# SamsungLabs/cloud_transformers

Hardware: AMD Instinct MI355X
Metric: points/sec fwd+bwd MHCT, 4096-pt batch, 1/2/4/8 MI355X; % HBM roofline (higher is better)
Workload: dtype f32; 1 GPU; north-star op-level: B=8 clouds x N=4096 pts, H=64 heads, C=16 feat/head, 2D grid W=32, reduce=max, keys=tanh(randn), seed 1234+rank; step = Splat fwd, Slice fwd, Slice bwd, Splat bwd (key cotangents summed); per_gpu_batch=8, parallelism=replica-sharded clouds x1 (no collective), world_size_seen=1, hip_graph=True, steps_per_graph=10

## Files before the change

### cloud_transformers_amd/csrc/ct_raster_bwd_fused.h

```cpp
#pragma once

typedef unsigned ct_u4 __attribute__((ext_vector_type(4)));
struct StreamBuf {
  __amdgpu_buffer_rsrc_t r;
};
constexpr int kBufNt = 2;
__device__ __forceinline__ StreamBuf stream_buf(const float* base, unsigned bytes) {
  StreamBuf b;
  b.r = __builtin_amdgcn_make_buffer_rsrc((void*)base, 0, (int)bytes, 0x00020000);
  return b;
}
__device__ __forceinline__ float4 buf_ld_stream4(const StreamBuf& b, unsigned voff, unsigned soff) {
  const ct_u4 v = __builtin_amdgcn_raw_buffer_load_b128(b.r, (int)voff, (int)soff, kBufNt);
  return make_float4(__uint_as_float(v.x), __uint_as_float(v.y), __uint_as_float(v.z), __uint_as_float(v.w));
}
__device__ __forceinline__ float buf_ld_stream(const StreamBuf& b, unsigned voff, unsigned soff) {
  return __uint_as_float(__builtin_amdgcn_raw_buffer_load_b32(b.r, (int)voff, (int)soff, kBufNt));
}
__device__ __forceinline__ void buf_st_stream4(const StreamBuf& b, unsigned voff, unsigned soff, float4 v) {
  const ct_u4 t = {__float_as_uint(v.x), __float_as_uint(v.y), __float_as_uint(v.z), __float_as_uint(v.w)};
  __builtin_amdgcn_raw_buffer_store_b128(t, b.r, (int)voff, (int)soff, kBufNt);
}
__device__ __forceinline__ void buf_st_stream(const StreamBuf& b, unsigned voff, unsigned soff, float v) {
  __builtin_amdgcn_raw_buffer_store_b32(__float_as_uint(v), b.r, (int)voff, (int)soff, kBufNt);
}

template <bool HAS_PAD, int WT, int NT = 0, int CT = 0>
__global__ void __launch_bounds__(kSortThreads) slice_splat_bwd_kernel(RasterArgs a_arg, GridW<2> g_arg) {
  const GridW<2> g = grid2_of<WT>(g_arg);
  RasterArgs a = a_arg;
  if constexpr (NT > 0) a.N = NT;
  if constexpr (CT > 0) a.C = CT;
  extern __shared__ __align__(16) unsigned char lds_raw[];
  const int G = WT ? WT * WT : g.G, W1 = WT ? WT : g.W[1], N = a.N, C = a.C;
  const SortLds L = sort_lds(G, N, C);
  float4* T4 = (float4*)(lds_raw + L.tile);
  int* acc = (int*)(lds_raw + L.acc);
  float4* ZG = (float4*)(lds_raw + L.tile);
  float4* Sg = (float4*)(lds_raw + L.stage);
  const float2* AB = (const float2*)(lds_raw + L.ab);
  unsigned* s_max = (unsigned*)(lds_raw + L.misc);
  unsigned* s_k = s_max + C;
  int* s_tie = (int*)(s_k + 1);
  const int b = blockIdx.z;
  const size_t bh = (size_t)b * a.H + blockIdx.y;
  const int tid = threadIdx.x;
  const int off[4] = {0, W1, 1, W1 + 1};
  const bool has = (tid << 2) < N;
  const int n0 = has ? (tid << 2) : 0;
  const int ngroups = C >> 2;
  const float* const feat = a.tile_in2;

  float gq[4][4];
  float fq[4][4];
  float cvq[4];
  const unsigned ln0 = (unsigned)n0;
  const unsigned pt_row = (unsigned)N * 4u, cell_row = (unsigned)G * 4u;
  const StreamBuf b_src = stream_buf(a.src + bh * C * (size_t)N, (unsigned)C * pt_row);
  const StreamBuf b_fea = stream_buf(feat + bh * C * (size_t)N, (unsigned)C * pt_row);
  const StreamBuf b_dst = stream_buf(a.dst + bh * C * (size_t)N, (unsigned)C * pt_row);
  const StreamBuf b_cnv = stream_buf(a.tile_in + bh * C * (size_t)G, (unsigned)C * cell_row);
  const StreamBuf b_gz = stream_buf(a.tile_out + bh * C * (size_t)G, (unsigned)C * cell_row);
  const unsigned vo_pt = ln0 * 4u, vo_cell = tid < G ? (unsigned)tid * 4u : 0u;
  auto request1 = [&](int grp, int cj) {
    const float4 t = buf_ld_stream4(b_src, vo_pt, (unsigned)(grp * 4 + cj) * pt_row);
    gq[cj][0] = t.x; gq[cj][1] = t.y; gq[cj][2] = t.z; gq[cj][3] = t.w;
    cvq[cj] = buf_ld_stream(b_cnv, vo_cell, (unsigned)(grp * 4 + cj) * cell_row);
  };
  auto request_feat1 = [&](int grp, int cj) {
    const float4 t = buf_ld_stream4(b_fea, vo_pt, (unsigned)(grp * 4 + cj) * pt_row);
    fq[cj][0] = t.x; fq[cj][1] = t.y; fq[cj][2] = t.z; fq[cj][3] = t.w;
  };
  PlaneKeys PK;
  load_plane_keys(a, g, W1, bh, PK);
  SortedPlane S;
  float pv[4];
#pragma unroll
  for (int i = 0; i < 4; ++i) pv[i] = (HAS_PAD && has) ? ct_load_pad(a.pad, a.pad_dtype, (size_t)b * N + n0 + i) : 1.0f;

  sort_plane(a, PK, G, W1, sort_ptrs(lds_raw, L, C), C, S, nullptr, [&]() {
#pragma unroll
    for (int cj = 0; cj < 4; ++cj) request1(0, cj);
  });
  uint2* const s_cell = (uint2*)(lds_raw + L.mark);
  s_cell[tid] = make_uint2((unsigned)PK.base[0] | (unsigned)PK.base[1] << 16, (unsigned)PK.base[2] | (unsigned)PK.base[3] << 16);
  for (int i = tid; i < G; i += kSortThreads) ((int4*)acc)[i] = make_int4(0, 0, 0, 0);
  if (tid == 0) Sg[N] = make_float4(0.0f, 0.0f, 0.0f, 0.0f);
  if (tid < 4) s_tie[tid] = 0;
  const float Kf = (float)(*s_k);

  float gsx[2][kItemLen], gsy[2][kItemLen];
#pragma unroll
  for (int u = 0; u < 2; ++u)
#pragma unroll
    for (int j = 0; j < kItemLen; ++j) gsx[u][j] = gsy[u][j] = 0.0f;
  float gs[4][2];
#pragma unroll
  for (int i = 0; i < 4; ++i) gs[i][0] = gs[i][1] = 0.0f;
  unsigned cell01 = ((unsigned)S.cell[0] & 0xffffu) | (unsigned)S.cell[1] << 16;
  unsigned long long tied = 0ull;

  auto group = [&](const int grp, auto more) {
    const int ch0 = grp * 4;
    asm volatile("" : "+v"(S.rk01), "+v"(S.rk23), "+v"(cell01));
    const int cell[2] = {(int)(short)(cell01 & 0xffffu), (int)cell01 >> 16};
#pragma unroll
    for (int cj = 0; cj < 4; ++cj) {
      float m = 0.0f;
#pragma unroll
      for (int i = 0; i < 4; ++i) {
        float x = HAS_PAD ? gq[cj][i] * pv[i] : gq[cj][i];
        x = has ? x : 0.0f;
        gq[cj][i] = x;
        x = fabsf(x);
        m = fmaxf(m, (x < __builtin_inff()) ? x : __builtin_inff());
      }
      const unsigned mb = wave_max_u32(__float_as_uint(m));
      if ((tid & 63) == 0) atomicMax(&s_max[ch0 + cj], mb);
    }
    if (has) {
      const unsigned rk[4] = {S.rk01 & kRankMask, (S.rk01 >> 16) & kRankMask, S.rk23 & kRankMask, (S.rk23 >> 16) & kRankMask};
#pragma unroll
      for (int i = 0; i < 4; ++i) Sg[rk[i]] = make_float4(gq[0][i], gq[1][i], gq[2][i], gq[3][i]);
    }
    if (tid < G) T4[tid] = make_float4(cvq[0], cvq[1], cvq[2], cvq[3]);
    __syncthreads();

    float iq[4];
    bool any_float = false;
#pragma unroll
    for (int cj = 0; cj < 4; ++cj) {
      float q;
      bool fixed;
      fx_quantum(__uint_as_float(s_max[ch0 + cj]) * Kf, q, iq[cj], fixed);
      if (!fixed) {
        iq[cj] = 0.0f;
        any_float = true;
      }
      iq[cj] = __uint_as_float(__builtin_amdgcn_readfirstlane(__float_as_uint(iq[cj])));
    }
    auto item = [&](auto U) {
      constexpr int u = decltype(U)::value;
      int Y = cell[u] < 0 ? 0 : cell[u];
      asm volatile("" : "+v"(S.ent8[u][0]), "+v"(S.ent8[u][1]), "+v"(Y));
      float4 cv[4];
#pragma unroll
      for (int v = 0; v < 4; ++v) cv[v] = T4[Y + off[v]];
      float4 xn = *(const float4*)((const unsigned char*)Sg + 2u * CT_E8(S, u, 0));
      float2 wn = *(const float2*)((const unsigned char*)AB + CT_E8(S, u, 0));
      ct_f2 s01[4], s23[4];
#pragma unroll
      for (int v = 0; v < 4; ++v) s01[v] = s23[v] = ct_f2{0.0f, 0.0f};
#pragma unroll
      for (int j = 0; j < kItemLen; ++j) {
        if constexpr (u == 0) request_feat1(grp, j);
        const float4 x = xn;
        const float2 wf = wn;
        if (j + 1 < kItemLen) {
          xn = *(const float4*)((const unsigned char*)Sg + 2u * CT_E8(S, u, j + 1));
          wn = *(const float2*)((const unsigned char*)AB + CT_E8(S, u, j + 1));
        }
        const ct_f2 x01 = {x.x, x.y}, x23 = {x.z, x.w};
        const float w1x = wf.x, w1y = wf.y, w0x = 1.0f - w1x, w0y = 1.0f - w1y;
        const float cw[4] = {w0x * w0y, w1x * w0y, w0x * w1y, w1x * w1y};
        float gw[4];
#pragma unroll
        for (int v = 0; v < 4; ++v) {
          const ct_f2 cwv = {cw[v], cw[v]};
          s01[v] = __builtin_elementwise_fma(x01, cwv, s01[v]);
          s23[v] = __builtin_elementwise_fma(x23, cwv, s23[v]);
          const ct_f2 c01 = {cv[v].x, cv[v].y}, c23 = {cv[v].z, cv[v].w};
          const ct_f2 pr = __builtin_elementwise_fma(c23, x23, c01 * x01);
          gw[v] = pr.x + pr.y;
        }
        gsx[u][j] = __builtin_fmaf(gw[3] - gw[2], w1y, __builtin_fmaf(gw[1] - gw[0], w0y, gsx[u][j]));
        gsy[u][j] = __builtin_fmaf(gw[3] - gw[1], w1x, __builtin_fmaf(gw[2] - gw[0], w0x, gsy[u][j]));
        asm volatile("" : "+v"(gsx[u][j]), "+v"(gsy[u][j]));
        CT_SB;
      }
      if (cell[u] >= 0) {
        const ct_f2 iq01 = {iq[0], iq[1]}, iq23 = {iq[2], iq[3]};
        int* Tc = acc + Y;
#pragma unroll
        for (int v = 0; v < 4; ++v) {
          const ct_f2 a01 = s01[v] * iq01, a23 = s23[v] * iq23;
          atomicAdd(Tc + off[v], cvt_rpi(a01.x));
          atomicAdd(Tc + G + off[v], cvt_rpi(a01.y));
          atomicAdd(Tc + 2 * G + off[v], cvt_rpi(a23.x));
          atomicAdd(Tc + 3 * G + off[v], cvt_rpi(a23.y));
        }
      }
      CT_SB;
    };
    item(std::integral_constant<int, 0>{});
    if (cell[1] >= 0) item(std::integral_constant<int, 1>{});
    if (any_float) {
#pragma unroll 1
      for (int cj = 0; cj < 4; ++cj)
        if (iq[cj] == 0.0f) scatter_float_channel<HAS_PAD>(a, g, bh, b, ch0 + cj, (float*)(acc + cj * G), 1, 0);
    }
    __syncthreads();

    float4 zc = make_float4(0.0f, 0.0f, 0.0f, 0.0f);
    float gv[4] = {0.0f, 0.0f, 0.0f, 0.0f};
    if (tid < G) {
      zc = T4[tid];
#pragma unroll
      for (int cj = 0; cj < 4; ++cj) {
        float q, iqd;
        bool fixed;
        fx_quantum(__uint_as_float(s_max[ch0 + cj]) * Kf, q, iqd, fixed);
        const int r = acc[cj * G + tid];
        gv[cj] = fixed ? (float)r * q : __int_as_float(r);
        buf_st_stream(b_gz, vo_cell, (unsigned)(ch0 + cj) * cell_row, gv[cj]);
      }
    }
    const unsigned zw[4] = {__float_as_uint(zc.x), __float_as_uint(zc.y), __float_as_uint(zc.z), __float_as_uint(zc.w)};
    {
      int nzt = 0;
#pragma unroll
      for (int k = 0; k < 4; ++k) nzt += (zw[k] != 0u);
      nzt = wave_sum_i32(nzt);
      if ((tid & 63) == 0 && nzt) atomicAdd(&s_tie[(grp & 1) * 2], nzt);
    }
    __syncthreads();
    if (tid < G) {
      ZG[tid] = make_float4(__uint_as_float(zw[0] ? zw[0] : kNoMatch), __uint_as_float(zw[1] ? zw[1] : kNoMatch), gv[0], gv[1]);
      ZG[G + tid] = make_float4(__uint_as_float(zw[2] ? zw[2] : kNoMatch), __uint_as_float(zw[3] ? zw[3] : kNoMatch), gv[2], gv[3]);
    }
    __syncthreads();

    int nm = 0;
    if (has) {
      const uint2 bc = s_cell[tid];
      const unsigned rk[4] = {S.rk01 & kRankMask, (S.rk01 >> 16) & kRankMask, S.rk23 & kRankMask, (S.rk23 >> 16) & kRankMask};
      const int pbase[4] = {(int)(bc.x & 0xffffu), (int)(bc.x >> 16), (int)(bc.y & 0xffffu), (int)(bc.y >> 16)};
#pragma unroll
      for (int i = 0; i < 4; ++i) {
        if constexpr (decltype(more)::value) request1(grp + 1, i);
        const float2 w1 = AB[rk[i]];
        Pt2 p;
        p.w1x = w1.x; p.w1y = w1.y; p.w0x = 1.0f - w1.x; p.w0y = 1.0f - w1.y;
        p.base = pbase[i];
        p.cw[0] = p.w0x * p.w0y; p.cw[1] = p.w1x * p.w0y; p.cw[2] = p.w0x * p.w1y; p.cw[3] = p.w1x * p.w1y;
        float gw[4] = {0.0f, 0.0f, 0.0f, 0.0f};
#pragma unroll
        for (int pr = 0; pr < 2; ++pr) {
          const float4* Zp = ZG + (size_t)pr * G + p.base;
          const float xa = HAS_PAD ? fq[2 * pr][i] * pv[i] : fq[2 * pr][i];
          const float xb = HAS_PAD ? fq[2 * pr + 1][i] * pv[i] : fq[2 * pr + 1][i];
          ct_f4 zg[4];
#pragma unroll
          for (int v = 0; v < 4; ++v) zg[v] = *(const ct_f4*)(Zp + off[v]);
#pragma unroll
          for (int v = 0; v < 4; ++v) asm volatile("" : "+v"(zg[v].x), "+v"(zg[v].y), "+v"(zg[v].z), "+v"(zg[v].w));
          float gfa = 0.0f, gfb = 0.0f;
#pragma unroll
          for (int v = 0; v < 4; ++v) {
            const unsigned ba = __float_as_uint(xa * p.cw[v]), bb = __float_as_uint(xb * p.cw[v]);
            const bool ma = ba == __float_as_uint(zg[v].x), mb = bb == __float_as_uint(zg[v].y);
            nm += (int)ma;
            nm += (int)mb;
            asm volatile("" : "+v"(nm));
            const float ga = ma ? zg[v].z : 0.0f, gb = mb ? zg[v].w : 0.0f;
            gfa = __builtin_fmaf(ga, p.cw[v], gfa);
            gfb = __builtin_fmaf(gb, p.cw[v], gfb);
            gw[v] = __builtin_fmaf(gb, xb, __builtin_fmaf(ga, xa, gw[v]));
          }
          fq[2 * pr][i] = HAS_PAD ? gfa * pv[i] : gfa;
          fq[2 * pr + 1][i] = HAS_PAD ? gfb * pv[i] : gfb;
        }
        gs[i][0] = __builtin_fmaf(gw[3] - gw[2], p.w1y, __builtin_fmaf(gw[1] - gw[0], p.w0y, gs[i][0]));
        gs[i][1] = __builtin_fmaf(gw[3] - gw[1], p.w1x, __builtin_fmaf(gw[2] - gw[0], p.w0x, gs[i][1]));
        asm volatile("" : "+v"(gs[i][0]), "+v"(gs[i][1]), "+v"(fq[0][i]), "+v"(fq[1][i]), "+v"(fq[2][i]), "+v"(fq[3][i]));
        __builtin_amdgcn_sched_barrier(0);
      }
#pragma unroll
      for (int cj = 0; cj < 4; ++cj)
        buf_st_stream4(b_dst, vo_pt, (unsigned)(ch0 + cj) * pt_row, make_float4(fq[cj][0], fq[cj][1], fq[cj][2], fq[cj][3]));
    } else if constexpr (decltype(more)::value) {
#pragma unroll
      for (int cj = 0; cj < 4; ++cj) request1(grp + 1, cj);
    }
    nm = wave_sum_i32(nm);
    if ((tid & 63) == 0 && nm) atomicAdd(&s_tie[(grp & 1) * 2 + 1], nm);
    __syncthreads();
    const int* tw = s_tie + (grp & 1) * 2;
    if (tw[0] != tw[1]) tied |= 1ull << grp;
    if (tid < 2) s_tie[((grp & 1) ^ 1) * 2 + tid] = 0;
    int zero;
    asm volatile("v_mov_b32 %0, 0" : "=v"(zero));
    if (tid < G) ((int4*)acc)[tid] = make_int4(zero, zero, zero, zero);
  };
  int grp = 0;
  for (; grp + 1 < ngroups; ++grp) group(grp, std::true_type{});
  group(grp, std::false_type{});

  if (tied != 0ull) {
    __builtin_amdgcn_fence(__ATOMIC_RELEASE, "workgroup");
    asm volatile("s_waitcnt vmcnt(0)" ::: "memory");
    __syncthreads();
    __builtin_amdgcn_fence(__ATOMIC_ACQUIRE, "workgroup");
    RasterArgs a2 = a;
    a2.src = feat;
    PtRows R;
    R.Nr = N; R.so = 0; R.wt = false;
    for (int gi = 0; gi < ngroups; ++gi) {
      if (!((tied >> gi) & 1ull)) continue;
      const int cabs = gi << 2;
      const float* zin = a.tile_in + (bh * C + cabs) * (size_t)G;
      const float* gin = a.tile_out + (bh * C + cabs) * (size_t)G;
      __syncthreads();
      {
        int nz_unused = 0;
        unsigned long long nzp_unused = 0ull;
        unsigned xzp_unused = 0u;
        stage_tile_pairs<false>(ZG, zin, gin, 2, G, nz_unused, nzp_unused, xzp_unused);
      }
      __syncthreads();
      if (has) {
        const float* const key0 = a.pos.keys + bh * 2 * (size_t)N;
        const float4 tx = *(const float4*)(key0 + ln0), ty = *(const float4*)(key0 + N + ln0);
        const float kx[4] = {tx.x, tx.y, tx.z, tx.w}, ky[4] = {ty.x, ty.y, ty.z, ty.w};
        int nm_unused = 0;
        unsigned u0 = 0u, u1 = 0u;
        splat_bwd_quad<HAS_PAD, true, WT, true>(a2, g, ZG, bh, b, cabs, 4, n0, R, kx, ky, gs, nm_unused, u0, u1, false);
      }
    }
    __syncthreads();
  }

  float2* Gs = (float2*)Sg;
#pragma unroll
  for (int u = 0; u < 2; ++u)
#pragma unroll
    for (int j = 0; j < kItemLen; ++j)
      *(float2*)((unsigned char*)Gs + CT_E8(S, u, j)) = make_float2(gsx[u][j], gsy[u][j]);
  __syncthreads();
  if (has) {
    const unsigned rw[4] = {S.rk01 & 0xffffu, S.rk01 >> 16, S.rk23 & 0xffffu, S.rk23 >> 16};
    float2 gk[4];
#pragma unroll
    for (int i = 0; i < 4; ++i) {
      gk[i] = Gs[rw[i] & kRankMask];
      gk[i].x *= (rw[i] & kInsideX) ? 1.0f : 0.0f;
      gk[i].y *= (rw[i] & kInsideY) ? 1.0f : 0.0f;
    }
    if (a.fold_gpos != nullptr) {
      st_stream4(a.fold_gpos + (bh * 2 + 0) * N + n0, make_float4(gk[0].x, gk[1].x, gk[2].x, gk[3].x));
      st_stream4(a.fold_gpos + (bh * 2 + 1) * N + n0, make_float4(gk[0].y, gk[1].y, gk[2].y, gk[3].y));
    }
    float mx[4], my[4];
#pragma unroll
    for (int i = 0; i < 4; ++i) {
      mx[i] = (rw[i] & kInsideX) ? 1.0f : 0.0f;
      my[i] = (rw[i] & kInsideY) ? 1.0f : 0.0f;
    }
    float4 ox = make_float4(gs[0][0] * mx[0], gs[1][0] * mx[1], gs[2][0] * mx[2], gs[3][0] * mx[3]);
    float4 oy = make_float4(gs[0][1] * my[0], gs[1][1] * my[1], gs[2][1] * my[2], gs[3][1] * my[3]);
    ox.x += gk[0].x; ox.y += gk[1].x; ox.z += gk[2].x; ox.w += gk[3].x;
    oy.x += gk[0].y; oy.y += gk[1].y; oy.z += gk[2].y; oy.w += gk[3].y;
    *(float4*)(a.g_pos + (bh * 2 + 0) * N + n0) = ox;
    *(float4*)(a.g_pos + (bh * 2 + 1) * N + n0) = oy;
  }
}
```

Measured before the change: 212.9 million points/s.

## Add in-register tie repair path for fused slice/splat backward before slow fallback

Adds a fast repair routine for channel groups flagged as having max-reduce ties in the fused backward kernel. It rebuilds the tile in LDS and resolves tied cells with atomicMax claims over up to eight conflicts, correcting the per-point gradients in place. Only when it cannot resolve a group does it fall back to the existing path, which re-stages tile pairs from global memory and re-runs splat_bwd_quad. This adds LDS traffic, extra syncs and register pressure for tied groups. Some asm barriers on indices are also inserted to steer code generation.

```diff
diff --git a/cloud_transformers_amd/csrc/ct_raster_bwd_fused.h b/cloud_transformers_amd/csrc/ct_raster_bwd_fused.h
--- a/cloud_transformers_amd/csrc/ct_raster_bwd_fused.h
+++ b/cloud_transformers_amd/csrc/ct_raster_bwd_fused.h
@@ -23,6 +23,171 @@
 }
 __device__ __forceinline__ void buf_st_stream(const StreamBuf& b, unsigned voff, unsigned soff, float v) {
   __builtin_amdgcn_raw_buffer_store_b32(__float_as_uint(v), b.r, (int)voff, (int)soff, kBufNt);
+}
+
+constexpr int kFusedTieMax = 8;
+__device__ __forceinline__ int fused_tie_corner(int d, int W1) { return d == 0 ? 0 : d == W1 ? 1 : d == 1 ? 2 : d == W1 + 1 ? 3 : -1; }
+
+__device__ __forceinline__ bool fused_bwd_repair_group(float4* T4, int* claim, float4* G4, int* s_rep, const uint2* s_cell,
+                                                       const float2* AB, unsigned rk01, unsigned rk23, const StreamBuf& b_gz,
+                                                       const StreamBuf& b_dst, unsigned vo_pt, unsigned vo_cell, unsigned pt_row,
+                                                       unsigned cell_row, int cabs, int G, int W1, bool has, int n0,
+                                                       const float (&x)[4][4], const float (&zc)[4], float (&gs)[4][2]) {
+  constexpr int K = kFusedTieMax;
+  int tid = threadIdx.x;
+  asm volatile("" : "+v"(tid), "+v"(rk01), "+v"(rk23));
+  const int off[4] = {0, W1, 1, W1 + 1};
+  if (tid < 3 + K) s_rep[tid] = 0;
+  int cnt = 0;
+  if (tid < G) {
+    unsigned zw[4];
+#pragma unroll
+    for (int cj = 0; cj < 4; ++cj) {
+      zw[cj] = __float_as_uint(zc[cj]);
+      cnt += zw[cj] != 0u;
+      zw[cj] = zw[cj] ? zw[cj] : kNoMatch;
+    }
+    T4[tid] = make_float4(__uint_as_float(zw[0]), __uint_as_float(zw[1]), __uint_as_float(zw[2]), __uint_as_float(zw[3]));
+#pragma unroll
+    for (int cj = 0; cj < 4; ++cj) claim[cj * G + tid] = 0;
+  }
+  cnt = wave_sum_i32(cnt);
+  __syncthreads();
+  __builtin_amdgcn_fence(__ATOMIC_ACQUIRE, "workgroup");
+  if ((tid & 63) == 0 && cnt) atomicAdd(&s_rep[2], cnt);
+  float gq[4];
+#pragma unroll
+  for (int cj = 0; cj < 4; ++cj) gq[cj] = buf_ld_stream(b_gz, vo_cell, (unsigned)(cabs + cj) * cell_row);
+
+  const unsigned rk[4] = {rk01 & kRankMask, (rk01 >> 16) & kRankMask, rk23 & kRankMask, (rk23 >> 16) & kRankMask};
+  auto base_of = [&](int i) -> int {
+    const uint2 bc = s_cell[tid];
+    return (int)(i == 0 ? bc.x & 0xffffu : i == 1 ? bc.x >> 16 : i == 2 ? bc.y & 0xffffu : bc.y >> 16);
+  };
+  unsigned mlo = 0u, mhi = 0u;
+  if (has) {
+#pragma unroll
+    for (int i = 0; i < 4; ++i) {
+      const float2 w1 = AB[rk[i]];
+      const float w0x = 1.0f - w1.x, w0y = 1.0f - w1.y;
+      const float cw[4] = {w0x * w0y, w1.x * w0y, w0x * w1.y, w1.x * w1.y};
+      const float4* Zp = T4 + base_of(i);
+      unsigned mi = 0u;
+#pragma unroll
+      for (int v = 0; v < 4; ++v) {
+        const float4 z4 = Zp[off[v]];
+        const float zz[4] = {z4.x, z4.y, z4.z, z4.w};
+#pragma unroll
+        for (int cj = 0; cj < 4; ++cj)
+          mi = mi + mi + (unsigned)(__float_as_uint(x[cj][i] * cw[v]) == __float_as_uint(zz[cj]));
+      }
+      if (i < 2) mlo |= mi << (16 * i);
+      else mhi |= mi << (16 * (i - 2));
+      asm volatile("" : "+v"(mlo), "+v"(mhi));
+      __builtin_amdgcn_sched_barrier(0);
+    }
+  }
+  const unsigned long long mm = (unsigned long long)mhi << 32 | mlo;
+  cnt = 0;
+  if (has) {
+    cnt = __builtin_popcountll(mm);
+#pragma unroll 1
+    for (unsigned long long m = mm; m != 0ull; m &= m - 1ull) {
+      const int bit = __builtin_ctzll(m), i = bit >> 4, r = 15 - (bit & 15), v = r >> 2, ch = r & 3;
+      const int cell = base_of(i) + (v == 0 ? 0 : v == 1 ? W1 : v == 2 ? 1 : W1 + 1);
+      if (atomicMax(&claim[ch * G + cell], 0x7fffffff - (n0 + i)) != 0) {
+        const int k = atomicAdd(&s_rep[0], 1);
+        if (k < K) s_rep[3 + k] = cell | ch << 16;
+      }
+    }
+  }
+  cnt = wave_sum_i32(cnt);
+  if ((tid & 63) == 0 && cnt) atomicAdd(&s_rep[1], cnt);
+  if (tid < G) G4[tid] = make_float4(gq[0], gq[1], gq[2], gq[3]);
+  __syncthreads();
+
+  const int L = s_rep[0];
+  if (L > K || L != s_rep[1] - s_rep[2]) return false;
+
+  auto match_bit = [&](int i, int cell, int ch) -> int {
+    const int v = fused_tie_corner(cell - base_of(i), W1);
+    return v < 0 ? -1 : 16 * i + 15 - (4 * v + ch);
+  };
+  unsigned long long lost = 0ull;
+  if (has && mm != 0ull) {
+#pragma unroll 1
+    for (int k = 0; k < L; ++k) {
+      const int e = s_rep[3 + k], win = 0x7fffffff - claim[(e >> 16) * G + (e & 0xffff)];
+#pragma unroll
+      for (int i = 0; i < 4; ++i) {
+        const int bit = match_bit(i, e & 0xffff, e >> 16);
+        if (bit >= 0 && ((mm >> bit) & 1ull) && win != n0 + i) lost |= 1ull << bit;
+      }
+    }
+  }
+  if (lost != 0ull) {
+    int prev = -1;
+#pragma unroll 1
+    for (;;) {
+      int e = 0x7fffffff;
+      for (int k = 0; k < L; ++k) {
+        const int ek = s_rep[3 + k];
+        e = (ek > prev && ek < e) ? ek : e;
+      }
+      if (e == 0x7fffffff) break;
+      prev = e;
+      const int cell = e & 0xffff, ch = e >> 16;
+#pragma unroll
+      for (int i = 0; i < 4; ++i) {
+        const int bit = match_bit(i, cell, ch);
+        if (bit < 0 || !((lost >> bit) & 1ull)) continue;
+        const float4 g4 = G4[cell];
+        const float gt = ch == 0 ? g4.x : ch == 1 ? g4.y : ch == 2 ? g4.z : g4.w;
+        const int vt = fused_tie_corner(cell - base_of(i), W1);
+        if (__float_as_uint(gt) == 0u) continue;
+        float gwt = 0.0f;
+#pragma unroll
+        for (int pr = 0; pr < 2; ++pr) {
+          const float da = ch == 2 * pr ? -gt : 0.0f, db = ch == 2 * pr + 1 ? -gt : 0.0f;
+          gwt = __builtin_fmaf(db, x[2 * pr + 1][i], __builtin_fmaf(da, x[2 * pr][i], gwt));
+        }
+        float gw[4];
+#pragma unroll
+        for (int v = 0; v < 4; ++v) gw[v] = v == vt ? gwt : 0.0f;
+        const float2 w1 = AB[rk[i]];
+        const float w0x = 1.0f - w1.x, w0y = 1.0f - w1.y;
+        const float d0 = __builtin_fmaf(gw[3] - gw[2], w1.y, (gw[1] - gw[0]) * w0y);
+        const float d1 = __builtin_fmaf(gw[3] - gw[1], w1.x, (gw[2] - gw[0]) * w0x);
+        gs[i][0] += d0;
+        gs[i][1] += d1;
+      }
+    }
+#pragma unroll
+    for (int i = 0; i < 4; ++i) {
+      const unsigned li = (unsigned)(lost >> (16 * i)) & 0xffffu;
+      if (li == 0u) continue;
+      const unsigned keep = (unsigned)(mm >> (16 * i)) & 0xffffu & ~li;
+      const float2 w1 = AB[rk[i]];
+      const float w0x = 1.0f - w1.x, w0y = 1.0f - w1.y;
+      const float cw[4] = {w0x * w0y, w1.x * w0y, w0x * w1.y, w1.x * w1.y};
+      const int pb = base_of(i);
+#pragma unroll
+      for (int cj = 0; cj < 4; ++cj) {
+        const unsigned chbits = 0x1111u << (3 - cj);
+        if (!(li & chbits)) continue;
+        float gf = 0.0f;
+#pragma unroll
+        for (int v = 0; v < 4; ++v) {
+          const float4 g4 = G4[pb + off[v]];
+          const float gc = cj == 0 ? g4.x : cj == 1 ? g4.y : cj == 2 ? g4.z : g4.w;
+          const bool won = (keep >> (15 - (4 * v + cj))) & 1u;
+          gf = __builtin_fmaf(won ? gc : 0.0f, cw[v], gf);
+        }
+        buf_st_stream(b_dst, vo_pt + 4u * (unsigned)i, (unsigned)(cabs + cj) * pt_row, gf);
+      }
+    }
+  }
+  return true;
 }
 
 template <bool HAS_PAD, int WT, int NT = 0, int CT = 0>
@@ -296,6 +461,45 @@
   for (; grp + 1 < ngroups; ++grp) group(grp, std::true_type{});
   group(grp, std::false_type{});
 
+  if constexpr (!HAS_PAD) {
+    if (tied != 0ull) {
+      float xq[4][4], zq[4];
+      int tq = tid;
+      asm volatile("" : "+v"(tq));
+      const unsigned vo_pt_c = has ? (unsigned)tq * 16u : 0u, vo_cell_c = tq < G ? (unsigned)tq * 4u : 0u;
+      auto request_tied = [&](int gi) {
+#pragma unroll
+        for (int cj = 0; cj < 4; ++cj) {
+          float4 t = make_float4(0.0f, 0.0f, 0.0f, 0.0f);
+          if (has) t = buf_ld_stream4(b_fea, vo_pt_c, (unsigned)(gi * 4 + cj) * pt_row);
+          xq[cj][0] = t.x; xq[cj][1] = t.y; xq[cj][2] = t.z; xq[cj][3] = t.w;
+          zq[cj] = buf_ld_stream(b_cnv, vo_cell_c, (unsigned)(gi * 4 + cj) * cell_row);
+        }
+      };
+      unsigned long long todo = tied;
+      tied = 0ull;
+      int gi = __builtin_ctzll(todo);
+      request_tied(gi);
+      __builtin_amdgcn_fence(__ATOMIC_RELEASE, "workgroup");
+      asm volatile("s_waitcnt vmcnt(0)" ::: "memory");
+#pragma unroll 1
+      for (;;) {
+        CT_TIE_COUNT(11, 1);
+        if (fused_bwd_repair_group(T4, acc, Sg, s_tie + 4, s_cell, AB, S.rk01, S.rk23, b_gz, b_dst, vo_pt_c, vo_cell_c, pt_row, cell_row,
+                                   gi << 2, G, W1, has, n0, xq, zq, gs)) {
+          CT_TIE_COUNT(12, 1);
+        } else {
+          tied |= 1ull << gi;
+        }
+        todo &= todo - 1ull;
+        if (todo == 0ull) break;
+        gi = __builtin_ctzll(todo);
+        request_tied(gi);
+        __syncthreads();
+      }
+      __syncthreads();
+    }
+  }
   if (tied != 0ull) {
     __builtin_amdgcn_fence(__ATOMIC_RELEASE, "workgroup");
     asm volatile("s_waitcnt vmcnt(0)" ::: "memory");
@@ -310,6 +514,7 @@
       const int cabs = gi << 2;
       const float* zin = a.tile_in + (bh * C + cabs) * (size_t)G;
       const float* gin = a.tile_out + (bh * C + cabs) * (size_t)G;
+      CT_TIE_COUNT(13, 1);
       __syncthreads();
       {
         int nz_unused = 0;
@@ -320,7 +525,9 @@
       __syncthreads();
       if (has) {
         const float* const key0 = a.pos.keys + bh * 2 * (size_t)N;
-        const float4 tx = *(const float4*)(key0 + ln0), ty = *(const float4*)(key0 + N + ln0);
+        unsigned lnr = ln0;
+        asm volatile("" : "+v"(lnr));
+        const float4 tx = *(const float4*)(key0 + lnr), ty = *(const float4*)(key0 + N + lnr);
         const float kx[4] = {tx.x, tx.y, tx.z, tx.w}, ky[4] = {ty.x, ty.y, ty.z, ty.w};
         int nm_unused = 0;
         unsigned u0 = 0u, u1 = 0u;
@@ -338,6 +545,8 @@
       *(float2*)((unsigned char*)Gs + CT_E8(S, u, j)) = make_float2(gsx[u][j], gsy[u][j]);
   __syncthreads();
   if (has) {
+    int n0s = n0;
+    asm volatile("" : "+v"(n0s));
     const unsigned rw[4] = {S.rk01 & 0xffffu, S.rk01 >> 16, S.rk23 & 0xffffu, S.rk23 >> 16};
     float2 gk[4];
 #pragma unroll
@@ -347,8 +556,8 @@
       gk[i].y *= (rw[i] & kInsideY) ? 1.0f : 0.0f;
     }
     if (a.fold_gpos != nullptr) {
-      st_stream4(a.fold_gpos + (bh * 2 + 0) * N + n0, make_float4(gk[0].x, gk[1].x, gk[2].x, gk[3].x));
-      st_stream4(a.fold_gpos + (bh * 2 + 1) * N + n0, make_float4(gk[0].y, gk[1].y, gk[2].y, gk[3].y));
+      st_stream4(a.fold_gpos + (bh * 2 + 0) * N + n0s, make_float4(gk[0].x, gk[1].x, gk[2].x, gk[3].x));
+      st_stream4(a.fold_gpos + (bh * 2 + 1) * N + n0s, make_float4(gk[0].y, gk[1].y, gk[2].y, gk[3].y));
     }
     float mx[4], my[4];
 #pragma unroll
@@ -360,7 +569,7 @@
     float4 oy = make_float4(gs[0][1] * my[0], gs[1][1] * my[1], gs[2][1] * my[2], gs[3][1] * my[3]);
     ox.x += gk[0].x; ox.y += gk[1].x; ox.z += gk[2].x; ox.w += gk[3].x;
     oy.x += gk[0].y; oy.y += gk[1].y; oy.z += gk[2].y; oy.w += gk[3].y;
-    *(float4*)(a.g_pos + (bh * 2 + 0) * N + n0) = ox;
-    *(float4*)(a.g_pos + (bh * 2 + 1) * N + n0) = oy;
-  }
-}
+    *(float4*)(a.g_pos + (bh * 2 + 0) * N + n0s) = ox;
+    *(float4*)(a.g_pos + (bh * 2 + 1) * N + n0s) = oy;
+  }
+}
```

After: 212.1 million points/s. About the same (-0.4%).

## Drop a barrier in fused slice/splat backward via separate staging buffer and row reductions

Applied to the files above, without the earlier changes.

Cross-lane reductions for the channel max and the tie counters now use 16-lane DPP row reductions, with atomics issued from each row's last lane instead of full-wave reductions with one atomic per wave. The zero/gradient tile for the slice backward is written into the stage region (PZ) rather than aliasing the tile buffer. This removes one __syncthreads per channel group, and the accumulator is cleared inline where it is read. The dequantisation scale is derived from the already broadcast inverse quantum by exponent arithmetic instead of recomputing fx_quantum, and the asm register pins are skipped for fixed-width tiles. In exchange there are 4x more LDS atomics, and correctness relies on PZ not overlapping Sg or AB data that is still live.

```diff
diff --git a/cloud_transformers_amd/csrc/ct_raster_bwd_fused.h b/cloud_transformers_amd/csrc/ct_raster_bwd_fused.h
--- a/cloud_transformers_amd/csrc/ct_raster_bwd_fused.h
+++ b/cloud_transformers_amd/csrc/ct_raster_bwd_fused.h
@@ -23,6 +23,27 @@
 }
 __device__ __forceinline__ void buf_st_stream(const StreamBuf& b, unsigned voff, unsigned soff, float v) {
   __builtin_amdgcn_raw_buffer_store_b32(__float_as_uint(v), b.r, (int)voff, (int)soff, kBufNt);
+}
+
+__device__ __forceinline__ unsigned row_max_u32(unsigned v) {
+#define CT_UMAX(a, b) max((a), (b))
+  CT_DPP_STEP(v, CT_UMAX, 0x111, 0xf);
+  CT_DPP_STEP(v, CT_UMAX, 0x112, 0xf);
+  CT_DPP_STEP(v, CT_UMAX, 0x114, 0xf);
+  CT_DPP_STEP(v, CT_UMAX, 0x118, 0xf);
+#undef CT_UMAX
+  asm volatile("" : "+v"(v));
+  return v;
+}
+__device__ __forceinline__ int row_sum_i32(int v) {
+#define CT_IADD(a, b) ((a) + (b))
+  CT_DPP_STEP(v, CT_IADD, 0x111, 0xf);
+  CT_DPP_STEP(v, CT_IADD, 0x112, 0xf);
+  CT_DPP_STEP(v, CT_IADD, 0x114, 0xf);
+  CT_DPP_STEP(v, CT_IADD, 0x118, 0xf);
+#undef CT_IADD
+  asm volatile("" : "+v"(v));
+  return v;
 }
 
 template <bool HAS_PAD, int WT, int NT = 0, int CT = 0>
@@ -42,6 +63,8 @@
   unsigned* s_max = (unsigned*)(lds_raw + L.misc);
   unsigned* s_k = s_max + C;
   int* s_tie = (int*)(s_k + 1);
+  float4* PZ = (float4*)(lds_raw + L.stage);
+  const bool row_last = (threadIdx.x & 15) == 15;
   const int b = blockIdx.z;
   const size_t bh = (size_t)b * a.H + blockIdx.y;
   const int tid = threadIdx.x;
@@ -85,7 +108,6 @@
   uint2* const s_cell = (uint2*)(lds_raw + L.mark);
   s_cell[tid] = make_uint2((unsigned)PK.base[0] | (unsigned)PK.base[1] << 16, (unsigned)PK.base[2] | (unsigned)PK.base[3] << 16);
   for (int i = tid; i < G; i += kSortThreads) ((int4*)acc)[i] = make_int4(0, 0, 0, 0);
-  if (tid == 0) Sg[N] = make_float4(0.0f, 0.0f, 0.0f, 0.0f);
   if (tid < 4) s_tie[tid] = 0;
   const float Kf = (float)(*s_k);
 
@@ -104,6 +126,11 @@
     const int ch0 = grp * 4;
     asm volatile("" : "+v"(S.rk01), "+v"(S.rk23), "+v"(cell01));
     const int cell[2] = {(int)(short)(cell01 & 0xffffu), (int)cell01 >> 16};
+    unsigned rowmax[4];
+    unsigned lane0;
+    asm volatile("v_mov_b32 %0, 0" : "=v"(lane0));
+    unsigned* const s_max_lane = s_max + lane0;
+    int* const s_tie_lane = s_tie + lane0;
 #pragma unroll
     for (int cj = 0; cj < 4; ++cj) {
       float m = 0.0f;
@@ -115,9 +142,13 @@
         x = fabsf(x);
         m = fmaxf(m, (x < __builtin_inff()) ? x : __builtin_inff());
       }
-      const unsigned mb = wave_max_u32(__float_as_uint(m));
-      if ((tid & 63) == 0) atomicMax(&s_max[ch0 + cj], mb);
-    }
+      rowmax[cj] = row_max_u32(__float_as_uint(m));
+    }
+    if (row_last) {
+#pragma unroll
+      for (int cj = 0; cj < 4; ++cj) atomicMax(s_max_lane + ch0 + cj, rowmax[cj]);
+    }
+    if (tid == 0) Sg[N] = make_float4(0.0f, 0.0f, 0.0f, 0.0f);
     if (has) {
       const unsigned rk[4] = {S.rk01 & kRankMask, (S.rk01 >> 16) & kRankMask, S.rk23 & kRankMask, (S.rk23 >> 16) & kRankMask};
 #pragma unroll
@@ -126,7 +157,7 @@
     if (tid < G) T4[tid] = make_float4(cvq[0], cvq[1], cvq[2], cvq[3]);
     __syncthreads();
 
-    float iq[4];
+    float iq[4], qs[4];
     bool any_float = false;
 #pragma unroll
     for (int cj = 0; cj < 4; ++cj) {
@@ -138,6 +169,7 @@
         any_float = true;
       }
       iq[cj] = __uint_as_float(__builtin_amdgcn_readfirstlane(__float_as_uint(iq[cj])));
+      qs[cj] = __uint_as_float(0x7f000000u - __float_as_uint(iq[cj]));
     }
     auto item = [&](auto U) {
       constexpr int u = decltype(U)::value;
@@ -207,26 +239,23 @@
       zc = T4[tid];
 #pragma unroll
       for (int cj = 0; cj < 4; ++cj) {
-        float q, iqd;
-        bool fixed;
-        fx_quantum(__uint_as_float(s_max[ch0 + cj]) * Kf, q, iqd, fixed);
         const int r = acc[cj * G + tid];
-        gv[cj] = fixed ? (float)r * q : __int_as_float(r);
+        gv[cj] = iq[cj] != 0.0f ? (float)r * qs[cj] : __int_as_float(r);
         buf_st_stream(b_gz, vo_cell, (unsigned)(ch0 + cj) * cell_row, gv[cj]);
+        acc[cj * G + tid] = 0;
       }
     }
     const unsigned zw[4] = {__float_as_uint(zc.x), __float_as_uint(zc.y), __float_as_uint(zc.z), __float_as_uint(zc.w)};
+    if (tid < G) {
+      PZ[tid] = make_float4(__uint_as_float(zw[0] ? zw[0] : kNoMatch), __uint_as_float(zw[1] ? zw[1] : kNoMatch), gv[0], gv[1]);
+      PZ[G + tid] = make_float4(__uint_as_float(zw[2] ? zw[2] : kNoMatch), __uint_as_float(zw[3] ? zw[3] : kNoMatch), gv[2], gv[3]);
+    }
     {
       int nzt = 0;
 #pragma unroll
       for (int k = 0; k < 4; ++k) nzt += (zw[k] != 0u);
-      nzt = wave_sum_i32(nzt);
-      if ((tid & 63) == 0 && nzt) atomicAdd(&s_tie[(grp & 1) * 2], nzt);
-    }
-    __syncthreads();
-    if (tid < G) {
-      ZG[tid] = make_float4(__uint_as_float(zw[0] ? zw[0] : kNoMatch), __uint_as_float(zw[1] ? zw[1] : kNoMatch), gv[0], gv[1]);
-      ZG[G + tid] = make_float4(__uint_as_float(zw[2] ? zw[2] : kNoMatch), __uint_as_float(zw[3] ? zw[3] : kNoMatch), gv[2], gv[3]);
+      nzt = row_sum_i32(nzt);
+      if (row_last && nzt) atomicAdd(s_tie_lane + (grp & 1) * 2, nzt);
     }
     __syncthreads();
 
@@ -246,14 +275,16 @@
         float gw[4] = {0.0f, 0.0f, 0.0f, 0.0f};
 #pragma unroll
         for (int pr = 0; pr < 2; ++pr) {
-          const float4* Zp = ZG + (size_t)pr * G + p.base;
+          const float4* Zp = PZ + (size_t)pr * G + p.base;
           const float xa = HAS_PAD ? fq[2 * pr][i] * pv[i] : fq[2 * pr][i];
           const float xb = HAS_PAD ? fq[2 * pr + 1][i] * pv[i] : fq[2 * pr + 1][i];
           ct_f4 zg[4];
 #pragma unroll
           for (int v = 0; v < 4; ++v) zg[v] = *(const ct_f4*)(Zp + off[v]);
-#pragma unroll
-          for (int v = 0; v < 4; ++v) asm volatile("" : "+v"(zg[v].x), "+v"(zg[v].y), "+v"(zg[v].z), "+v"(zg[v].w));
+          if constexpr (WT == 0) {
+#pragma unroll
+            for (int v = 0; v < 4; ++v) asm volatile("" : "+v"(zg[v].x), "+v"(zg[v].y), "+v"(zg[v].z), "+v"(zg[v].w));
+          }
           float gfa = 0.0f, gfb = 0.0f;
 #pragma unroll
           for (int v = 0; v < 4; ++v) {
@@ -282,15 +313,12 @@
 #pragma unroll
       for (int cj = 0; cj < 4; ++cj) request1(grp + 1, cj);
     }
-    nm = wave_sum_i32(nm);
-    if ((tid & 63) == 0 && nm) atomicAdd(&s_tie[(grp & 1) * 2 + 1], nm);
+    nm = row_sum_i32(nm);
+    if (row_last && nm) atomicAdd(s_tie_lane + (grp & 1) * 2 + 1, nm);
     __syncthreads();
     const int* tw = s_tie + (grp & 1) * 2;
     if (tw[0] != tw[1]) tied |= 1ull << grp;
     if (tid < 2) s_tie[((grp & 1) ^ 1) * 2 + tid] = 0;
-    int zero;
-    asm volatile("v_mov_b32 %0, 0" : "=v"(zero));
-    if (tid < G) ((int4*)acc)[tid] = make_int4(zero, zero, zero, zero);
   };
   int grp = 0;
   for (; grp + 1 < ngroups; ++grp) group(grp, std::true_type{});
```

Result: faster. 217.3 million points/s before, 223.0 million points/s after (median of 6 runs) (+2.6%).
